# aghasemzadeh/OpenMPL

Hardware: AMD Instinct MI355X
Metric: poses/sec (V=4, J=17, batch=1024 per GPU) fp32 (higher is better)
Workload: dtype f32; 1 GPU; Human3.6M config: V=4 J=17 batch=1024 fp32, CHOSEN flag set, depth 12, DIM 32, heads 8; global_batch=1024, parallelism=single GPU

## Files before the change

### openmpl_amd/csrc/spt.hip

```cpp
#include <stdlib.h>

#include "common.hpp"

namespace mpl {

constexpr int SJ = 17;
constexpr int SD = 32;
constexpr int SH = 8;
constexpr int SEQ = 16;
constexpr int ROWS = SEQ * SJ;
constexpr int MT = ROWS / 16;
constexpr int XS = 36;
constexpr int QS = 100;
constexpr int NTHR = 512;
constexpr int NWAVE = NTHR / 64;
constexpr int SPT_LDS_BYTES = (ROWS * XS + ROWS * QS) * 4;

struct SptParams {
    const float* poses[MPL_MAX_VIEWS];
    const float* rays[MPL_MAX_VIEWS];
    const float* centers[MPL_MAX_VIEWS];
    const mpl_spt_set* sets;
    const float *snorm_w, *snorm_b;
    const float *pos3d_embed, *pos3d_view, *pos3d_lin_w, *pos3d_lin_b;
    const float *ray_w, *ray_b, *cfpt_w, *cfpt_b;
    float* xs;
    int B, V, in_ch, n_apps;
    unsigned flags;
    int c3;
    int spw;
    int abl;
    unsigned* err_host;
    unsigned char sched[MPL_MAX_APPS];
};

typedef const __attribute__((address_space(1))) float* gfp;
__device__ __forceinline__ gfp G(const float* p) { return (gfp)p; }
__device__ __forceinline__ float4 ld4(gfp p) {
    typedef float v4 __attribute__((ext_vector_type(4)));
    const v4 t = *reinterpret_cast<const __attribute__((address_space(1))) v4*>(p);
    return make_float4(t.x, t.y, t.z, t.w);
}

__device__ __forceinline__ void ln_frags(const float* X, int m, int li, int kq, const float4& g0, const float4& g1,
                                         const float4& b0, const float4& b1, float4& a0, float4& a1) {
    const float* xr = X + (m * 16 + li) * XS + 4 * kq;
    float4 x0 = ld4(xr), x1 = ld4(xr + 16);
    float s = ((x0.x + x0.y) + (x0.z + x0.w)) + ((x1.x + x1.y) + (x1.z + x1.w));
    s = xor16_add(s);
    s = xor32_add(s);
    const float mean = s * (1.0f / 32.0f);
    x0.x -= mean; x0.y -= mean; x0.z -= mean; x0.w -= mean;
    x1.x -= mean; x1.y -= mean; x1.z -= mean; x1.w -= mean;
    float ss = ((x0.x * x0.x + x0.y * x0.y) + (x0.z * x0.z + x0.w * x0.w)) +
               ((x1.x * x1.x + x1.y * x1.y) + (x1.z * x1.z + x1.w * x1.w));
    ss = xor16_add(ss);
    ss = xor32_add(ss);
    const float rstd = 1.0f / sqrtf(ss * (1.0f / 32.0f) + 1e-6f);
    a0.x = x0.x * rstd * g0.x + b0.x; a0.y = x0.y * rstd * g0.y + b0.y;
    a0.z = x0.z * rstd * g0.z + b0.z; a0.w = x0.w * rstd * g0.w + b0.w;
    a1.x = x1.x * rstd * g1.x + b1.x; a1.y = x1.y * rstd * g1.y + b1.y;
    a1.z = x1.z * rstd * g1.z + b1.z; a1.w = x1.w * rstd * g1.w + b1.w;
}

struct BlockFrags {
    float4 wq[6][2]; float bq[6];
    float4 wp[2][2]; float bp[2];
    float4 w1[4][2]; float b1[4];
    float4 w2[2][4]; float b2[2];
    float4 g1a, g1b, e1a, e1b;
    float4 g2a, g2b, e2a, e2b;
};

__device__ __forceinline__ void load_qkv_frags(const mpl_block_weights& bw, BlockFrags& F, int li, int kq) {
    F.g1a = ld4(G(bw.ln1_w) + 4 * kq); F.g1b = ld4(G(bw.ln1_w) + 16 + 4 * kq);
    F.e1a = ld4(G(bw.ln1_b) + 4 * kq); F.e1b = ld4(G(bw.ln1_b) + 16 + 4 * kq);
#pragma unroll
    for (int n = 0; n < 6; ++n) {
        const gfp wr = G(bw.qkv_w) + (n * 16 + li) * SD + 4 * kq;
        F.wq[n][0] = ld4(wr);
        F.wq[n][1] = ld4(wr + 16);
        F.bq[n] = G(bw.qkv_b)[n * 16 + li];
    }
}

__device__ __forceinline__ void load_proj_frags(const mpl_block_weights& bw, BlockFrags& F, int li, int kq) {
#pragma unroll
    for (int n = 0; n < 2; ++n) {
        const gfp wr = G(bw.proj_w) + (n * 16 + li) * SD + 4 * kq;
        F.wp[n][0] = ld4(wr);
        F.wp[n][1] = ld4(wr + 16);
        F.bp[n] = G(bw.proj_b)[n * 16 + li];
    }
}

__device__ __forceinline__ void load_fc1_frags(const mpl_block_weights& bw, BlockFrags& F, int li, int kq) {
    F.g2a = ld4(G(bw.ln2_w) + 4 * kq); F.g2b = ld4(G(bw.ln2_w) + 16 + 4 * kq);
    F.e2a = ld4(G(bw.ln2_b) + 4 * kq); F.e2b = ld4(G(bw.ln2_b) + 16 + 4 * kq);
#pragma unroll
    for (int n = 0; n < 4; ++n) {
        const gfp wr = G(bw.fc1_w) + (n * 16 + li) * SD + 4 * kq;
        F.w1[n][0] = ld4(wr);
        F.w1[n][1] = ld4(wr + 16);
        F.b1[n] = G(bw.fc1_b)[n * 16 + li];
    }
}

__device__ __forceinline__ void load_fc2_frags(const mpl_block_weights& bw, BlockFrags& F, int li, int kq) {
#pragma unroll
    for (int n = 0; n < 2; ++n) {
        const gfp wr = G(bw.fc2_w) + (n * 16 + li) * (2 * SD) + 4 * kq;
#pragma unroll
        for (int q = 0; q < 4; ++q) F.w2[n][q] = ld4(wr + 16 * q);
        F.b2[n] = G(bw.fc2_b)[n * 16 + li];
    }
}

constexpr int SPT_WB_VEC = 8192;
constexpr int SPT_WB_FLOATS = SPT_WB_VEC + 512;
constexpr int SPT_SMALL_ROWS = 144;
constexpr int SPT_SMALL_SPW = 8;
constexpr int SPT_SMALL_LDS_BYTES = (SPT_SMALL_ROWS * (XS + QS) + 2 * SPT_WB_FLOATS) * 4;
__device__ __forceinline__ const float* spt_uniform(const float* q) {
    const unsigned long long v = (unsigned long long)(uintptr_t)q;
    const unsigned lo = __builtin_amdgcn_readfirstlane((unsigned)v), hi = __builtin_amdgcn_readfirstlane((unsigned)(v >> 32));
    return reinterpret_cast<const float*>((uintptr_t)(((unsigned long long)hi << 32) | lo));
}
__device__ __forceinline__ void stage_block(const mpl_block_weights& bwv, float* wb, int wave, int lane, int w0, int nw) {
    if (wave < w0 || wave >= w0 + nw) return;
    const int li = lane & 15, kq = lane >> 4;
    struct { const float *qkv_w, *proj_w, *fc1_w, *fc2_w, *qkv_b, *proj_b, *fc1_b, *fc2_b, *ln1_w, *ln1_b, *ln2_w, *ln2_b; } bw;
    bw.qkv_w = spt_uniform(bwv.qkv_w); bw.proj_w = spt_uniform(bwv.proj_w); bw.fc1_w = spt_uniform(bwv.fc1_w); bw.fc2_w = spt_uniform(bwv.fc2_w);
    bw.qkv_b = spt_uniform(bwv.qkv_b); bw.proj_b = spt_uniform(bwv.proj_b); bw.fc1_b = spt_uniform(bwv.fc1_b); bw.fc2_b = spt_uniform(bwv.fc2_b);
    bw.ln1_w = spt_uniform(bwv.ln1_w); bw.ln1_b = spt_uniform(bwv.ln1_b); bw.ln2_w = spt_uniform(bwv.ln2_w); bw.ln2_b = spt_uniform(bwv.ln2_b);
    const unsigned lds0 = __builtin_amdgcn_readfirstlane((unsigned)(uintptr_t)(__attribute__((address_space(3))) float*)wb);
    for (int pc = wave - w0; pc < 34; pc += nw) {
        const float* src;
        bool on = true;
        if (pc < 12) src = bw.qkv_w + ((pc >> 1) * 16 + li) * SD + 16 * (pc & 1) + 4 * kq;
        else if (pc < 16) src = bw.proj_w + (((pc - 12) >> 1) * 16 + li) * SD + 16 * (pc & 1) + 4 * kq;
        else if (pc < 24) src = bw.fc1_w + (((pc - 16) >> 1) * 16 + li) * SD + 16 * (pc & 1) + 4 * kq;
        else if (pc < 32) src = bw.fc2_w + (((pc - 24) >> 2) * 16 + li) * (2 * SD) + 16 * (pc & 3) + 4 * kq;
        else if (pc == 32)
            src = lane < 24 ? bw.qkv_b + 4 * lane
                : lane < 32 ? bw.proj_b + 4 * (lane - 24)
                : lane < 48 ? bw.fc1_b + 4 * (lane - 32)
                : lane < 56 ? bw.fc2_b + 4 * (lane - 48) : bw.ln1_w + 4 * (lane - 56);
        else {
            src = lane < 8 ? bw.ln1_b + 4 * lane : lane < 16 ? bw.ln2_w + 4 * (lane - 8) : bw.ln2_b + 4 * (lane - 16);
            on = lane < 24;
        }
        if (on) dma16(src, lds0 + (unsigned)(pc * 1024));
    }
// ... 269 lines not shown
#pragma unroll
            for (int j = 0; j < SJ; ++j) {
                const float4 v = ld4(kb + j * QS + SD);
                const float pj = sc[j] * inv;
                o.x = fmaf(pj, v.x, o.x);
                o.y = fmaf(pj, v.y, o.y);
                o.z = fmaf(pj, v.z, o.z);
                o.w = fmaf(pj, v.w, o.w);
            }
            st4(Q + r * QS + 4 * h, o);
        }
        __syncthreads();
        stamp(1);

        if (!STAGED) {
#pragma unroll
            for (int n = 0; n < 2; ++n) { touch(F.wp[n][0]); touch(F.wp[n][1]); touch(F.bp[n]); }
            load_fc1_frags(bw, F, li, kq);
        }
        if (STAGED) {
            const int lo = (mt * 2 * wave) / NWAVE, hi = (mt * 2 * (wave + 1)) / NWAVE;
            for (int u = lo; u < hi && !(p.abl & 4); ++u) {
                const int m = u >> 1, n = u & 1;
                const float4 w0 = wb4(wb, 12 + 2 * n, lane), w1 = wb4(wb, 12 + 2 * n + 1, lane);
                const float bp = wb[SPT_WB_VEC + 96 + n * 16 + li];
                const float* ar = Q + (m * 16 + li) * QS + 4 * kq;
                const float4 a0 = ld4(ar), a1 = ld4(ar + 16);
                const f32x4 c = tile_k32(a0, a1, w0, w1);
                float* xd = X + (m * 16 + 4 * kq) * XS + n * 16 + li;
#pragma unroll
                for (int r = 0; r < 4; ++r) xd[r * XS] += c[r] + bp;
            }
        } else {
            const int lo = (mt * 2 * wave) / NWAVE, hi = (mt * 2 * (wave + 1)) / NWAVE;
            for (int m = lo >> 1; m <= ((hi - 1) >> 1) && !(p.abl & 4); ++m) {
                const float* ar = Q + (m * 16 + li) * QS + 4 * kq;
                const float4 a0 = ld4(ar), a1 = ld4(ar + 16);
#pragma unroll
                for (int n = 0; n < 2; ++n) {
                    const int u = 2 * m + n;
                    if (u < lo || u >= hi) continue;
                    const f32x4 c = tile_k32(a0, a1, F.wp[n][0], F.wp[n][1]);
                    float* xd = X + (m * 16 + 4 * kq) * XS + n * 16 + li;
#pragma unroll
                    for (int r = 0; r < 4; ++r) xd[r * XS] += c[r] + F.bp[n];
                }
            }
        }
        __syncthreads();
        stamp(2);

        if (!STAGED) {
#pragma unroll
            for (int n = 0; n < 4; ++n) { touch(F.w1[n][0]); touch(F.w1[n][1]); touch(F.b1[n]); }
            touch(F.g2a); touch(F.g2b); touch(F.e2a); touch(F.e2b);
            load_fc2_frags(bw, F, li, kq);
        }
        if (STAGED) {
            const int lo = (mt * 4 * wave) / NWAVE, hi = (mt * 4 * (wave + 1)) / NWAVE;
            const float4 g0 = wbv4(wb, 288, kq), g1 = wbv4(wb, 304, kq), e0 = wbv4(wb, 320, kq), e1 = wbv4(wb, 336, kq);
            float4 a0, a1;
            int m_have = -1;
            for (int u = lo; u < hi && !(p.abl & 4); ++u) {
                const int m = u >> 2, n = u & 3;
                const float4 w0 = wb4(wb, 16 + 2 * n, lane), w1 = wb4(wb, 16 + 2 * n + 1, lane);
                const float b1 = wb[SPT_WB_VEC + 128 + n * 16 + li];
                if (m != m_have) { ln_frags(X, m, li, kq, g0, g1, e0, e1, a0, a1); m_have = m; }
                const f32x4 c = tile_k32(a0, a1, w0, w1);
                float* qd = Q + (m * 16 + 4 * kq) * QS + n * 16 + li;
#pragma unroll
                for (int r = 0; r < 4; ++r) qd[r * QS] = (p.abl & 2) ? (c[r] + b1) : gelu_erf(c[r] + b1);
            }
        } else {
            const int lo = (mt * 4 * wave) / NWAVE, hi = (mt * 4 * (wave + 1)) / NWAVE;
            for (int m = lo >> 2; m <= ((hi - 1) >> 2) && !(p.abl & 4); ++m) {
                float4 a0, a1;
                ln_frags(X, m, li, kq, F.g2a, F.g2b, F.e2a, F.e2b, a0, a1);
#pragma unroll
                for (int n = 0; n < 4; ++n) {
                    const int u = 4 * m + n;
                    if (u < lo || u >= hi) continue;
                    const f32x4 c = tile_k32(a0, a1, F.w1[n][0], F.w1[n][1]);
                    float* qd = Q + (m * 16 + 4 * kq) * QS + n * 16 + li;
#pragma unroll
                    for (int r = 0; r < 4; ++r)
                        qd[r * QS] = (p.abl & 2) ? (c[r] + F.b1[n]) : gelu_erf(c[r] + F.b1[n]);
                }
            }
        }
        __syncthreads();
        stamp(3);

        if (!STAGED) {
#pragma unroll
            for (int n = 0; n < 2; ++n) {
#pragma unroll
                for (int q = 0; q < 4; ++q) touch(F.w2[n][q]);
                touch(F.b2[n]);
            }
            if (more) load_qkv_frags(bw_next, F, li, kq);
        }
        if (STAGED) {
            const int lo = (mt * 2 * wave) / NWAVE, hi = (mt * 2 * (wave + 1)) / NWAVE;
            for (int u = lo; u < hi && !(p.abl & 4); ++u) {
                const int m = u >> 1, n = u & 1;
                const float4 w0 = wb4(wb, 24 + 4 * n, lane), w1 = wb4(wb, 24 + 4 * n + 1, lane), w2 = wb4(wb, 24 + 4 * n + 2, lane),
                             w3 = wb4(wb, 24 + 4 * n + 3, lane);
                const float b2 = wb[SPT_WB_VEC + 192 + n * 16 + li];
                const float* ar = Q + (m * 16 + li) * QS + 4 * kq;
                const float4 a0 = ld4(ar), a1 = ld4(ar + 16), a2 = ld4(ar + 32), a3 = ld4(ar + 48);
                const f32x4 c = tile_k32(a0, a1, w0, w1) + tile_k32(a2, a3, w2, w3);
                float* xd = X + (m * 16 + 4 * kq) * XS + n * 16 + li;
#pragma unroll
                for (int r = 0; r < 4; ++r) xd[r * XS] += c[r] + b2;
            }
        } else {
            const int lo = (mt * 2 * wave) / NWAVE, hi = (mt * 2 * (wave + 1)) / NWAVE;
            for (int m = lo >> 1; m <= ((hi - 1) >> 1) && !(p.abl & 4); ++m) {
                const float* ar = Q + (m * 16 + li) * QS + 4 * kq;
                const float4 a0 = ld4(ar), a1 = ld4(ar + 16), a2 = ld4(ar + 32), a3 = ld4(ar + 48);
#pragma unroll
                for (int n = 0; n < 2; ++n) {
                    const int u = 2 * m + n;
                    if (u < lo || u >= hi) continue;
                    const f32x4 c = tile_k32(a0, a1, F.w2[n][0], F.w2[n][1]) + tile_k32(a2, a3, F.w2[n][2], F.w2[n][3]);
                    float* xd = X + (m * 16 + 4 * kq) * XS + n * 16 + li;
#pragma unroll
                    for (int r = 0; r < 4; ++r) xd[r * XS] += c[r] + F.b2[n];
                }
            }
        }
        if (STAGED) asm volatile("s_waitcnt vmcnt(0)" ::: "memory");
        __syncthreads();
        stamp(4);
        bw = bw_next;
        if (STAGED && app + 2 < p.n_apps) bw_next = bw_after;
    }

    if ((p.abl & 16) && lane == 0 && blockIdx.x < 32) {
        float* o = p.xs + (size_t)(blockIdx.x * NWAVE + wave) * 8;
        for (int k = 0; k < 6; ++k) o[k] = (float)ph[k];
        return;
    }
    if (p.abl & 16) return;
    spt_epilogue<false>(p, X, tid, view, b0, pose, ray, cen, nl, rows_live);
}

constexpr int ATS = 36;
constexpr int HS = 68;
constexpr int KV_F = SJ * SH * SEQ * 4;
constexpr int SPT3_RING_BYTES = (ROWS * XS + 2 * KV_F + ROWS * ATS) * 4;
constexpr int SPT3_LDS_BYTES = 160 * 1024;
constexpr int SPT3_HID_OFF = 3072;
constexpr int SPT3_Q_OFF = 20480;
constexpr int SPT3_NPAR = 456;
static_assert(SPT3_HID_OFF + ROWS * HS <= 2 * KV_F + ROWS * ATS, "HID does not fit its alias");
static_assert((SPT3_HID_OFF + ROWS * HS - 2 * KV_F) * 4 <= SPT3_Q_OFF, "HID reaches into the staged qkv weights");
static_assert(SPT3_Q_OFF + 12 * 1024 <= ROWS * ATS * 4, "staged qkv weights do not fit behind HID in ATT");
static_assert(SPT3_RING_BYTES + 8 * 1024 + 2 * SPT3_NPAR * 4 <= SPT3_LDS_BYTES, "spare LDS too small");
constexpr int SPT_PACK_QKV = 0, SPT_PACK_PROJ = 12 * 1024, SPT_PACK_FC1 = 16 * 1024, SPT_PACK_FC2 = 24 * 1024;
constexpr int SPT_PACK_VEC = 32 * 1024;
constexpr int SPT_PACK_BYTES = 48 * 1024;
constexpr int SPT_C_QKV = 0, SPT_C_PROJ = 96, SPT_C_FC1 = 128, SPT_C_FC2 = 192, SPT_NCOL = 224;
constexpr float SPT_SA = 1024.0f;
constexpr float SPT_QS = 0.5f * 1.4426950408889634f;

typedef _Float16 sf16x8 __attribute__((ext_vector_type(8)));
typedef float f32x2 __attribute__((ext_vector_type(2)));

__device__ __forceinline__ void spt_split2(const float (&x)[8], sf16x8& hi, sf16x8& lo) { ::mpl::split2_f16(x, hi, lo); }
__device__ inline float spt_window_scale(float v) {
    if (!(v > 0.f) || !(v < 3.0e38f)) return 1.0f;
    int e;
    (void)frexpf(32768.0f / v, &e);
    e = e - 1 < -100 ? -100 : (e - 1 > 100 ? 100 : e - 1);
    return ldexpf(1.0f, e);
}

__global__ __launch_bounds__(256) void spt_pack_kernel(const float* __restrict__ qkv_w, const float* __restrict__ qkv_b,
                                                        const float* __restrict__ ln1_w, const float* __restrict__ ln1_b,
                                                        const float* __restrict__ proj_w, const float* __restrict__ proj_b,
                                                        const float* __restrict__ fc1_w, const float* __restrict__ fc1_b,
                                                        const float* __restrict__ ln2_w, const float* __restrict__ ln2_b,
                                                        const float* __restrict__ fc2_w, const float* __restrict__ fc2_b,
                                                        char* __restrict__ dst, int fold_q) {
    __shared__ float Wf[8192];
    __shared__ float cn[SPT_NCOL], sw[SPT_NCOL], bnd[SPT_NCOL], scal[2];
    const int tid = threadIdx.x;
    for (int i = tid; i < 8192; i += 256) {
        float w;
        if (i < 3072) w = qkv_w[i] * ln1_w[i & 31];
        else if (i < 4096) w = proj_w[i - 3072];
        else if (i < 6144) w = fc1_w[i - 4096] * ln2_w[i & 31];
        else w = fc2_w[i - 6144];
        Wf[i] = w;
    }
    __syncthreads();
    if (tid < SPT_NCOL) {
        const int n = tid;
        const float *wr, *raw, *beta = nullptr;
        int K = 32;
        float bias;
        if (n < 96) { wr = Wf + n * 32; raw = qkv_w + n * 32; beta = ln1_b; bias = qkv_b[n]; }
        else if (n < 128) { wr = Wf + 3072 + (n - 96) * 32; raw = proj_w + (n - 96) * 32; bias = proj_b[n - 96]; }
        else if (n < 192) { wr = Wf + 4096 + (n - 128) * 32; raw = fc1_w + (n - 128) * 32; beta = ln2_b; bias = fc1_b[n - 128]; }
        else { wr = Wf + 6144 + (n - 192) * 64; raw = fc2_w + (n - 192) * 64; bias = fc2_b[n - 192]; K = 64; }
        float amax = 0.f;
        double ss = 0.0, c = (double)bias;
        for (int k = 0; k < K; ++k) {
            amax = fmaxf(amax, fabsf(wr[k]));
            ss += (double)wr[k] * (double)wr[k];
            if (beta) c += (double)raw[k] * (double)beta[k];
        }
        float s = 1.0f;
        if (amax > 0.f && amax < 3.0e38f) {
            int e;
            (void)frexpf(amax, &e);
            e = 14 - e;
            e = e < -100 ? -100 : (e > 100 ? 100 : e);
            s = ldexpf(1.0f, e);
        }
        cn[n] = (float)c;
        sw[n] = s;
        bnd[n] = beta ? (float)(sqrt(32.0) * sqrt(ss)) + fabsf((float)c) : 0.f;
    }
    __syncthreads();
    if (tid == 0) {
        float batt = 0.f, bhid = 0.f;
        for (int n = 64; n < 96; ++n) batt = fmaxf(batt, bnd[n]);
        for (int n = SPT_C_FC1; n < SPT_C_FC2; ++n) bhid = fmaxf(bhid, bnd[n]);
        scal[0] = spt_window_scale(batt);
        scal[1] = spt_window_scale(bhid);
    }
    __syncthreads();
    float* vec = reinterpret_cast<float*>(dst + SPT_PACK_VEC);
    if (tid < SPT_NCOL) {
        const int n = tid;
        float c = cn[n], sc;
        if (n < 96) sc = 1.0f / (SPT_SA * sw[n]);
        else if (n < 128) sc = 1.0f / (scal[0] * sw[n]);
        else if (n < 192) sc = 1.0f / (SPT_SA * sw[n]);
        else sc = 1.0f / (scal[1] * sw[n]);
        if (n < 32 && fold_q) { c *= SPT_QS; sc *= SPT_QS; }
        vec[n] = c;
        vec[SPT_NCOL + n] = sc;
    }
    if (tid < 8) vec[2 * SPT_NCOL + tid] = tid == 0 ? scal[0] : (tid == 1 ? 0.5f * scal[1] : 0.f);
    sf16x8* frag = reinterpret_cast<sf16x8*>(dst);
    for (int idx = tid; idx < 16 * 64; idx += 256) {
        const int lane = idx & 63, u = idx >> 6, li = lane & 15, kq = lane >> 4;
        const float* src;
        int n;
        if (u < 6) { n = 16 * u + li; src = Wf + n * 32 + 8 * kq; }
        else if (u < 8) { n = 16 * (u - 6) + li; src = Wf + 3072 + n * 32 + 8 * kq; n += SPT_C_PROJ; }
        else if (u < 12) { n = 16 * (u - 8) + li; src = Wf + 4096 + n * 32 + 8 * kq; n += SPT_C_FC1; }
        else { n = 16 * ((u - 12) >> 1) + li; src = Wf + 6144 + n * 64 + 32 * ((u - 12) & 1) + 8 * kq; n += SPT_C_FC2; }
        float x[8];
#pragma unroll
        for (int j = 0; j < 8; ++j) x[j] = src[j] * sw[n];
        sf16x8 hi, lo;
        spt_split2(x, hi, lo);
        frag[(size_t)(u * 2) * 64 + lane] = hi;
        frag[(size_t)(u * 2 + 1) * 64 + lane] = lo;
    }
}

int launch_spt_pack(const mpl_block_weights* bw_host, unsigned short* dst, int fold_q, hipStream_t s) {
    const mpl_block_weights* b = bw_host;
    if (!b || !dst || !b->qkv_w || !b->proj_w || !b->fc1_w || !b->fc2_w || !b->qkv_b || !b->proj_b || !b->fc1_b || !b->fc2_b ||
        !b->ln1_w || !b->ln1_b || !b->ln2_w || !b->ln2_b)
        return MPL_E_INVALID;
    ProfScope prof(MPL_K_PACK, s);
    hipLaunchKernelGGL(spt_pack_kernel, dim3(1), dim3(256), 0, s, b->qkv_w, b->qkv_b, b->ln1_w, b->ln1_b, b->proj_w, b->proj_b, b->fc1_w,
                       b->fc1_b, b->ln2_w, b->ln2_b, b->fc2_w, b->fc2_b, reinterpret_cast<char*>(dst), fold_q);
    return hip_check_launch();
}

size_t spt_pack_bytes() { return SPT_PACK_BYTES; }

__device__ __forceinline__ f32x4 mfma3(const sf16x8 (&w)[2], const sf16x8& ah, const sf16x8& al, f32x4 c) {
    c = __builtin_amdgcn_mfma_f32_16x16x32_f16(w[0], al, c, 0, 0, 0);
    c = __builtin_amdgcn_mfma_f32_16x16x32_f16(w[1], ah, c, 0, 0, 0);
    c = __builtin_amdgcn_mfma_f32_16x16x32_f16(w[0], ah, c, 0, 0, 0);
    return c;
}

template <int SS>
__global__ __launch_bounds__(NTHR, 1) void spt3_kernel(const SptParams p) {
    constexpr int RLIVE = SJ * SS;
    constexpr int MTS = (RLIVE + 15) / 16;
    constexpr int NT = (MTS + 3) / 4;
    extern __shared__ __attribute__((aligned(16))) float smem[];
    float* X = smem;
    float* Kb = smem + ROWS * XS;
    float* Vb = Kb + KV_F;
    float* ATT = Vb + KV_F;
    float* HID = Kb + SPT3_HID_OFF;
    char* S_W = reinterpret_cast<char*>(ATT + ROWS * ATS);
    float* S_PAR = reinterpret_cast<float*>(S_W + 8 * 1024);
    char* R_F1 = reinterpret_cast<char*>(Kb);
    char* R_Q = reinterpret_cast<char*>(ATT) + SPT3_Q_OFF;

    const int tid = threadIdx.x, lane = tid & 63;
    const int wave = __builtin_amdgcn_readfirstlane(tid >> 6);
    const int li = lane & 15, kq = lane >> 4;
    auto phase_sync = [&]() {
        asm volatile("s_waitcnt vmcnt(0)" ::: "memory");
        __syncthreads();
    };
    const int hg = wave & 1, part = wave >> 1;
    const int view = blockIdx.x % p.V;
    const int b0 = (blockIdx.x / p.V) * SS;
    const int sl = li % SS;
    const mpl_spt_set set = p.sets[(p.flags & MPL_F_MULTI_SPT) ? view : 0];
    const float* pose = p.poses[view];
    const float* ray = p.rays[view];
    const float* cen = p.centers[view];

    auto stage_w = [&](char* dst, const unsigned short* pack, int byte_off, int n_pieces) {
        const unsigned l0 = (unsigned)(uintptr_t)(__attribute__((address_space(3))) char*)dst;
        for (int i = wave; i < n_pieces; i += NWAVE)
            ::mpl::dma16(reinterpret_cast<const float*>(reinterpret_cast<const char*>(pack) + byte_off + i * 1024) + lane * 4,
                         l0 + (unsigned)(i * 1024));
    };
    auto load_par = [&](const mpl_block_weights& b) -> float4 {
        if (tid >= SPT3_NPAR / 4) return float4{0.f, 0.f, 0.f, 0.f};
        return ld4(G(reinterpret_cast<const float*>(reinterpret_cast<const char*>(b.qkv_w3) + SPT_PACK_VEC)) + 4 * tid);
    };
    auto store_par = [&](int app_of, const float4& v) {
        if (tid < SPT3_NPAR / 4) st4(S_PAR + (app_of & 1) * SPT3_NPAR + 4 * tid, v);
    };
    mpl_block_weights bw;
    if (p.n_apps > 0) {
        bw = set.blocks[p.sched[0] & 0x7f];
        stage_w(R_Q, bw.qkv_w3, SPT_PACK_QKV, 12);
    }
    const float4 par0 = p.n_apps > 0 ? load_par(bw) : float4{0.f, 0.f, 0.f, 0.f};
    spt_embed<true, SS>(p, set, X, tid, b0, pose, ray, cen, SS, MTS * 16);
    store_par(0, par0);
    phase_sync();

    auto load_w = [&](const char* region, int unit, sf16x8 (&w)[2]) {
        const sf16x8* g = reinterpret_cast<const sf16x8*>(region) + (size_t)unit * 2 * 64 + lane;
        w[0] = g[0];
        w[1] = g[64];
    };
    auto ln_frag = [&](int m, sf16x8& ah, sf16x8& al) {
        const float* xr = X + (m * 16 + li) * XS + 8 * kq;
        float4 x0 = ::mpl::ld4(xr), x1 = ::mpl::ld4(xr + 4);
        float sm = ((x0.x + x0.y) + (x0.z + x0.w)) + ((x1.x + x1.y) + (x1.z + x1.w));
        sm = ::mpl::xor32_add(::mpl::xor16_add(sm));
        const float mean = sm * (1.0f / 32.0f);
        x0.x -= mean; x0.y -= mean; x0.z -= mean; x0.w -= mean;
        x1.x -= mean; x1.y -= mean; x1.z -= mean; x1.w -= mean;
        float ss = ((x0.x * x0.x + x0.y * x0.y) + (x0.z * x0.z + x0.w * x0.w)) +
                   ((x1.x * x1.x + x1.y * x1.y) + (x1.z * x1.z + x1.w * x1.w));
        ss = ::mpl::xor32_add(::mpl::xor16_add(ss));
        const float rs = __builtin_amdgcn_rsqf(ss * (1.0f / 32.0f) + 1e-6f) * SPT_SA;
        const float y[8] = {x0.x * rs, x0.y * rs, x0.z * rs, x0.w * rs, x1.x * rs, x1.y * rs, x1.z * rs, x1.w * rs};
        spt_split2(y, ah, al);
    };
    auto raw_frag = [&](const float* rowp, sf16x8& ah, sf16x8& al) {
        const float4 x0 = ::mpl::ld4(rowp), x1 = ::mpl::ld4(rowp + 4);
        const float y[8] = {x0.x, x0.y, x0.z, x0.w, x1.x, x1.y, x1.z, x1.w};
        spt_split2(y, ah, al);
    };

    for (int app = 0; app < p.n_apps; ++app) {
        const bool weighted = (p.sched[app] & 0x80) != 0;
        bw = set.blocks[p.sched[app] & 0x7f];
        const unsigned short* pack = bw.qkv_w3;
        const float* par = S_PAR + (app & 1) * SPT3_NPAR;
        stage_w(S_W, pack, SPT_PACK_PROJ, 4);
        {
            sf16x8 wq[3][2];
            float4 bq[3], sq[3];
#pragma unroll
            for (int c = 0; c < 3; ++c) {
                load_w(R_Q, 2 * c + hg, wq[c]);
                bq[c] = ::mpl::ld4(par + SPT_C_QKV + 32 * c + 16 * hg + 4 * kq);
                sq[c] = ::mpl::ld4(par + SPT_NCOL + SPT_C_QKV + 32 * c + 16 * hg + 4 * kq);
            }
            float4 q[NT];
#pragma unroll
            for (int t = 0; t < NT; ++t) {
                q[t] = float4{0.f, 0.f, 0.f, 0.f};
                if (part + 4 * t < MTS && !(p.abl & 8)) {
                    const int m = part + 4 * t;
                    const int j = (16 * m + li) / SS;
                    const bool live = 16 * m + li < RLIVE;
                    sf16x8 ah, al;
                    ln_frag(m, ah, al);
                    const f32x4 z = {0.f, 0.f, 0.f, 0.f};
                    const f32x4 cq = mfma3(wq[0], ah, al, z), ck = mfma3(wq[1], ah, al, z), cv = mfma3(wq[2], ah, al, z);
                    q[t] = float4{fmaf(cq[0], sq[0].x, bq[0].x), fmaf(cq[1], sq[0].y, bq[0].y), fmaf(cq[2], sq[0].z, bq[0].z),
                                  fmaf(cq[3], sq[0].w, bq[0].w)};
                    const int h = 4 * hg + kq;
                    const float kx = fmaf(ck[0], sq[1].x, bq[1].x), ky = fmaf(ck[1], sq[1].y, bq[1].y);
                    const float kz = fmaf(ck[2], sq[1].z, bq[1].z), kw = fmaf(ck[3], sq[1].w, bq[1].w);
                    if (live && j < SJ - 1) {
                        float* kp = Kb + ((((j >> 1) * 2) * SH + h) * SS + sl) * 4 + (j & 1);
                        kp[0] = kx;
                        kp[2] = ky;
                        kp[SH * SS * 4] = kz;
                        kp[SH * SS * 4 + 2] = kw;
                    } else if (live) {
                        st4(Kb + (SJ - 1) * SH * SS * 4 + (h * SS + sl) * 4, float4{kx, ky, kz, kw});
                    }
                    if (live)
                        st4(Vb + ((j * SH + h) * SS + sl) * 4, float4{fmaf(cv[0], sq[2].x, bq[2].x), fmaf(cv[1], sq[2].y, bq[2].y),
                                                                       fmaf(cv[2], sq[2].z, bq[2].z), fmaf(cv[3], sq[2].w, bq[2].w)});
                }
            }
            phase_sync();
            if (!(p.abl & 1)) {
                const int h = 4 * hg + kq;
                float sc[NT][SJ];
#pragma unroll
                for (int jp = 0; jp < SJ / 2; ++jp) {
                    const float4 k01 = ::mpl::ld4(Kb + (((jp * 2) * SH + h) * SS + sl) * 4);
                    const float4 k23 = ::mpl::ld4(Kb + (((jp * 2 + 1) * SH + h) * SS + sl) * 4);
                    const f32x2 kx = {k01.x, k01.y}, ky = {k01.z, k01.w}, kz = {k23.x, k23.y}, kw = {k23.z, k23.w};
#pragma unroll
                    for (int t = 0; t < NT; ++t) {
                        const f32x2 qx = {q[t].x, q[t].x}, qy = {q[t].y, q[t].y}, qz = {q[t].z, q[t].z}, qw = {q[t].w, q[t].w};
                        f32x2 s2 = qx * kx;
                        s2 = __builtin_elementwise_fma(qy, ky, s2);
                        s2 = __builtin_elementwise_fma(qz, kz, s2);
                        s2 = __builtin_elementwise_fma(qw, kw, s2);
                        sc[t][2 * jp] = s2[0];
                        sc[t][2 * jp + 1] = s2[1];
                    }
                }
                {
                    const float4 k = ::mpl::ld4(Kb + (SJ - 1) * SH * SS * 4 + (h * SS + sl) * 4);
#pragma unroll
                    for (int t = 0; t < NT; ++t)
                        sc[t][SJ - 1] = fmaf(q[t].w, k.w, fmaf(q[t].z, k.z, fmaf(q[t].y, k.y, q[t].x * k.x)));
                }
                const float s_att = par[2 * SPT_NCOL];
                float inv[NT];
#pragma unroll
                for (int t = 0; t < NT; ++t) {
                    float mx = sc[t][0];
#pragma unroll
                    for (int j = 1; j < SJ; ++j) mx = fmaxf(mx, sc[t][j]);
                    float l = 0.f;
#pragma unroll
                    for (int j = 0; j < SJ; ++j) {
                        sc[t][j] = __builtin_amdgcn_exp2f(sc[t][j] - mx);
                        l += sc[t][j];
                    }
                    inv[t] = __builtin_amdgcn_rcpf(l) * s_att;
                    if (weighted) {
                        const int b = b0 + sl, r = 16 * (part + 4 * t) + li;
                        inv[t] *= (b < p.B && r < RLIVE) ? pose[((size_t)b * SJ + r / SS) * 3 + 2] : 0.f;
                    }
                }
                float4 o[NT];
#pragma unroll
                for (int t = 0; t < NT; ++t) o[t] = float4{0.f, 0.f, 0.f, 0.f};
#pragma unroll
                for (int j = 0; j < SJ; ++j) {
                    const float4 v = ::mpl::ld4(Vb + ((j * SH + h) * SS + sl) * 4);
#pragma unroll
                    for (int t = 0; t < NT; ++t) {
                        const float pj = sc[t][j];
                        o[t].x = fmaf(pj, v.x, o[t].x);
                        o[t].y = fmaf(pj, v.y, o[t].y);
                        o[t].z = fmaf(pj, v.z, o[t].z);
                        o[t].w = fmaf(pj, v.w, o[t].w);
                    }
                }
#pragma unroll
                for (int t = 0; t < NT; ++t) {
                    o[t] = float4{o[t].x * inv[t], o[t].y * inv[t], o[t].z * inv[t], o[t].w * inv[t]};
                    if (weighted) {
                        const float big = fmaxf(fmaxf(fabsf(o[t].x), fabsf(o[t].y)), fmaxf(fabsf(o[t].z), fabsf(o[t].w)));
                        if (!(big <= 65000.f)) {
                            const float qn = __builtin_nanf("");
                            o[t] = float4{qn, qn, qn, qn};
                            if (p.err_host) __hip_atomic_fetch_or(p.err_host, 2u, __ATOMIC_RELAXED, __HIP_MEMORY_SCOPE_SYSTEM);
                        }
                    }
                }
#pragma unroll
                for (int t = 0; t < NT; ++t)
                    if (part + 4 * t < MTS) st4(ATT + ((part + 4 * t) * 16 + li) * ATS + 4 * h, o[t]);
            }
        }
        phase_sync();
        {
            stage_w(R_F1, pack, SPT_PACK_FC1, 8);
            sf16x8 wp[2][2];
            float4 bp[2], sp[2];
#pragma unroll
            for (int n = 0; n < 2; ++n) {
                load_w(S_W, n, wp[n]);
                bp[n] = ::mpl::ld4(par + SPT_C_PROJ + 16 * n + 4 * kq);
                sp[n] = ::mpl::ld4(par + SPT_NCOL + SPT_C_PROJ + 16 * n + 4 * kq);
            }
            const int lo = (MTS * 2 * wave) / NWAVE, hi = (MTS * 2 * (wave + 1)) / NWAVE;
            for (int m = lo >> 1; m <= ((hi - 1) >> 1) && !(p.abl & 32); ++m) {
                sf16x8 ah, al;
                raw_frag(ATT + (m * 16 + li) * ATS + 8 * kq, ah, al);
#pragma unroll
                for (int n = 0; n < 2; ++n) {
                    const int u = 2 * m + n;
                    if (u < lo || u >= hi) continue;
                    const f32x4 c = mfma3(wp[n], ah, al, f32x4{0.f, 0.f, 0.f, 0.f});
                    float* xd = X + (m * 16 + li) * XS + 16 * n + 4 * kq;
                    const float4 x = ::mpl::ld4(xd);
                    st4(xd, float4{x.x + fmaf(c[0], sp[n].x, bp[n].x), x.y + fmaf(c[1], sp[n].y, bp[n].y),
                                   x.z + fmaf(c[2], sp[n].z, bp[n].z), x.w + fmaf(c[3], sp[n].w, bp[n].w)});
                }
            }
        }
        phase_sync();
        {
            stage_w(S_W, pack, SPT_PACK_FC2, 8);
            sf16x8 w1[4][2];
            float4 b1[4], s1[4];
#pragma unroll
            for (int n = 0; n < 4; ++n) {
                load_w(R_F1, n, w1[n]);
                b1[n] = ::mpl::ld4(par + SPT_C_FC1 + 16 * n + 4 * kq);
                s1[n] = ::mpl::ld4(par + SPT_NCOL + SPT_C_FC1 + 16 * n + 4 * kq);
            }
            const float hs = par[2 * SPT_NCOL + 1];
            const int lo = (MTS * 4 * wave) / NWAVE, hi = (MTS * 4 * (wave + 1)) / NWAVE;
            for (int m = lo >> 2; m <= ((hi - 1) >> 2) && !(p.abl & 64); ++m) {
                sf16x8 ah, al;
                ln_frag(m, ah, al);
#pragma unroll
                for (int n = 0; n < 4; ++n) {
                    const int u = 4 * m + n;
                    if (u < lo || u >= hi) continue;
                    const f32x4 c = mfma3(w1[n], ah, al, f32x4{0.f, 0.f, 0.f, 0.f});
                    st4(HID + (m * 16 + li) * HS + 16 * n + 4 * kq,
                        float4{gelu_as_scaled(fmaf(c[0], s1[n].x, b1[n].x), hs), gelu_as_scaled(fmaf(c[1], s1[n].y, b1[n].y), hs),
                               gelu_as_scaled(fmaf(c[2], s1[n].z, b1[n].z), hs), gelu_as_scaled(fmaf(c[3], s1[n].w, b1[n].w), hs)});
                }
            }
        }
        phase_sync();
        {
            float4 parn = float4{0.f, 0.f, 0.f, 0.f};
            if (app + 1 < p.n_apps) {
                const mpl_block_weights bn = set.blocks[p.sched[app + 1] & 0x7f];
                stage_w(R_Q, bn.qkv_w3, SPT_PACK_QKV, 12);
                parn = load_par(bn);
            }
            sf16x8 w2[2][2][2];
            float4 b2[2], s2[2];
#pragma unroll
            for (int n = 0; n < 2; ++n) {
                load_w(S_W, 2 * n, w2[n][0]);
                load_w(S_W, 2 * n + 1, w2[n][1]);
                b2[n] = ::mpl::ld4(par + SPT_C_FC2 + 16 * n + 4 * kq);
                s2[n] = ::mpl::ld4(par + SPT_NCOL + SPT_C_FC2 + 16 * n + 4 * kq);
            }
            const int lo = (MTS * 2 * wave) / NWAVE, hi = (MTS * 2 * (wave + 1)) / NWAVE;
            for (int m = lo >> 1; m <= ((hi - 1) >> 1) && !(p.abl & 128); ++m) {
                sf16x8 ah0, al0, ah1, al1;
                raw_frag(HID + (m * 16 + li) * HS + 8 * kq, ah0, al0);
                raw_frag(HID + (m * 16 + li) * HS + 32 + 8 * kq, ah1, al1);
#pragma unroll
                for (int n = 0; n < 2; ++n) {
                    const int u = 2 * m + n;
                    if (u < lo || u >= hi) continue;
                    f32x4 c = mfma3(w2[n][0], ah0, al0, f32x4{0.f, 0.f, 0.f, 0.f});
                    c = mfma3(w2[n][1], ah1, al1, c);
                    float* xd = X + (m * 16 + li) * XS + 16 * n + 4 * kq;
                    const float4 x = ::mpl::ld4(xd);
                    st4(xd, float4{x.x + fmaf(c[0], s2[n].x, b2[n].x), x.y + fmaf(c[1], s2[n].y, b2[n].y),
                                   x.z + fmaf(c[2], s2[n].z, b2[n].z), x.w + fmaf(c[3], s2[n].w, b2[n].w)});
                }
            }
            if (app + 1 < p.n_apps) store_par(app + 1, parn);
        }
        phase_sync();
    }
    spt_epilogue<true, SS>(p, X, tid, view, b0, pose, ray, cen, SS, MTS * 16);
}

__device__ __forceinline__ void d32_ln_split(const float4& a0, const float4& a1, sf16x8& ah, sf16x8& al) {
    float4 x0 = a0, x1 = a1;
    float sm = ((x0.x + x0.y) + (x0.z + x0.w)) + ((x1.x + x1.y) + (x1.z + x1.w));
    sm = xor32_add(xor16_add(sm));
    const float mean = sm * (1.0f / 32.0f);
    x0.x -= mean; x0.y -= mean; x0.z -= mean; x0.w -= mean;
    x1.x -= mean; x1.y -= mean; x1.z -= mean; x1.w -= mean;
    float ss = ((x0.x * x0.x + x0.y * x0.y) + (x0.z * x0.z + x0.w * x0.w)) + ((x1.x * x1.x + x1.y * x1.y) + (x1.z * x1.z + x1.w * x1.w));
    ss = xor32_add(xor16_add(ss));
    const float rs = __builtin_amdgcn_rsqf(ss * (1.0f / 32.0f) + 1e-6f) * SPT_SA;
    const float y[8] = {x0.x * rs, x0.y * rs, x0.z * rs, x0.w * rs, x1.x * rs, x1.y * rs, x1.z * rs, x1.w * rs};
    spt_split2(y, ah, al);
}
__device__ __forceinline__ void d32_load_w(const char* pack, int unit, int lane, sf16x8 (&w)[2]) {
    const sf16x8* g = reinterpret_cast<const sf16x8*>(pack) + (size_t)unit * 2 * 64 + lane;
    w[0] = g[0];
    w[1] = g[64];
}

__global__ __launch_bounds__(512) void d32_qkv_kernel(const float* __restrict__ x, int M, const char* __restrict__ pack,
                                                       float* __restrict__ qkv) {
    const int lane = threadIdx.x & 63, li = lane & 15, kq = lane >> 4;
    const int gw = blockIdx.x * 8 + (threadIdx.x >> 6), nw = gridDim.x * 8;
    const float* vec = reinterpret_cast<const float*>(pack + SPT_PACK_VEC);
    sf16x8 wq[6][2];
    float4 cq[6], sq[6];
#pragma unroll
    for (int n = 0; n < 6; ++n) {
        d32_load_w(pack, n, lane, wq[n]);
        cq[n] = ld4(vec + SPT_C_QKV + 16 * n + 4 * kq);
        sq[n] = ld4(vec + SPT_NCOL + SPT_C_QKV + 16 * n + 4 * kq);
    }
    const int n_tiles = (M + 15) / 16;
    auto rows_of = [&](int tile, float4& a0, float4& a1) {
        const int r = tile * 16 + li;
        const float* xr = x + (size_t)(r < M ? r : M - 1) * SD + 8 * kq;
        a0 = ld4(xr);
        a1 = ld4(xr + 4);
    };
    float4 n0 = {0.f, 0.f, 0.f, 0.f}, n1 = n0;
    if (gw < n_tiles) rows_of(gw, n0, n1);
    for (int tile = gw; tile < n_tiles; tile += nw) {
        const int row = tile * 16 + li;
        const bool ok = row < M;
        const float4 c0 = n0, c1 = n1;
        if (tile + nw < n_tiles) rows_of(tile + nw, n0, n1);
        sf16x8 ah, al;
        d32_ln_split(c0, c1, ah, al);
        float* o = qkv + (size_t)row * (3 * SD) + 4 * kq;
#pragma unroll
        for (int n = 0; n < 6; ++n) {
            const f32x4 c = mfma3(wq[n], ah, al, f32x4{0.f, 0.f, 0.f, 0.f});
            if (ok) st4(o + 16 * n, float4{fmaf(c[0], sq[n].x, cq[n].x), fmaf(c[1], sq[n].y, cq[n].y), fmaf(c[2], sq[n].z, cq[n].z),
                                           fmaf(c[3], sq[n].w, cq[n].w)});
        }
    }
// ... 193 lines not shown
```

Measured before the change: 878,200 poses/s.

## Precompute LayerNorm fragments once into LDS and split attention by live tiles

Each wave now computes its share of LayerNorm fp16 hi/lo fragments once and stores them in the ATT region of LDS. The QKV staged weights move to the start of the K buffer to make room. Previously the fragments were recomputed redundantly by the head-group/part waves, and the QKV loop now reads them after an extra barrier. Attention is split into compile-time chunks of at most three tiles and dispatched by the number of live tiles per wave. This avoids computing dead tiles and lowers register pressure from the score arrays. The cost is an extra __syncthreads and changed LDS aliasing, which risks overlapping buffers.

```diff
diff --git a/openmpl_amd/csrc/spt.hip b/openmpl_amd/csrc/spt.hip
--- a/openmpl_amd/csrc/spt.hip
+++ b/openmpl_amd/csrc/spt.hip
@@ -1,4 +1,6 @@
 #include <stdlib.h>
+
+#include <type_traits>
 
 #include "common.hpp"
 
@@ -574,11 +576,10 @@
 constexpr int SPT3_RING_BYTES = (ROWS * XS + 2 * KV_F + ROWS * ATS) * 4;
 constexpr int SPT3_LDS_BYTES = 160 * 1024;
 constexpr int SPT3_HID_OFF = 3072;
-constexpr int SPT3_Q_OFF = 20480;
 constexpr int SPT3_NPAR = 456;
 static_assert(SPT3_HID_OFF + ROWS * HS <= 2 * KV_F + ROWS * ATS, "HID does not fit its alias");
-static_assert((SPT3_HID_OFF + ROWS * HS - 2 * KV_F) * 4 <= SPT3_Q_OFF, "HID reaches into the staged qkv weights");
-static_assert(SPT3_Q_OFF + 12 * 1024 <= ROWS * ATS * 4, "staged qkv weights do not fit behind HID in ATT");
+static_assert(12 * 1024 <= SPT3_HID_OFF * 4, "staged qkv weights reach into HID");
+static_assert(MT * 2048 <= ROWS * ATS * 4, "LayerNorm fragments do not fit in ATT");
 static_assert(SPT3_RING_BYTES + 8 * 1024 + 2 * SPT3_NPAR * 4 <= SPT3_LDS_BYTES, "spare LDS too small");
 constexpr int SPT_PACK_QKV = 0, SPT_PACK_PROJ = 12 * 1024, SPT_PACK_FC1 = 16 * 1024, SPT_PACK_FC2 = 24 * 1024;
 constexpr int SPT_PACK_VEC = 32 * 1024;
@@ -721,7 +722,8 @@
     char* S_W = reinterpret_cast<char*>(ATT + ROWS * ATS);
     float* S_PAR = reinterpret_cast<float*>(S_W + 8 * 1024);
     char* R_F1 = reinterpret_cast<char*>(Kb);
-    char* R_Q = reinterpret_cast<char*>(ATT) + SPT3_Q_OFF;
+    char* R_Q = reinterpret_cast<char*>(Kb);
+    sf16x8* FR = reinterpret_cast<sf16x8*>(ATT);
 
     const int tid = threadIdx.x, lane = tid & 63;
     const int wave = __builtin_amdgcn_readfirstlane(tid >> 6);
@@ -803,6 +805,19 @@
                 bq[c] = ::mpl::ld4(par + SPT_C_QKV + 32 * c + 16 * hg + 4 * kq);
                 sq[c] = ::mpl::ld4(par + SPT_NCOL + SPT_C_QKV + 32 * c + 16 * hg + 4 * kq);
             }
+            if (!(p.abl & 8)) {
+#pragma unroll
+                for (int i = 0; i < 3; ++i) {
+                    const int m = i < 2 ? wave + NWAVE * i : 2 * NWAVE + (NWAVE - 1 - wave);
+                    if (m < MTS) {
+                        sf16x8 ah, al;
+                        ln_frag(m, ah, al);
+                        FR[(2 * m) * 64 + lane] = ah;
+                        FR[(2 * m + 1) * 64 + lane] = al;
+                    }
+                }
+            }
+            __syncthreads();
             float4 q[NT];
 #pragma unroll
             for (int t = 0; t < NT; ++t) {
@@ -811,8 +826,7 @@
                     const int m = part + 4 * t;
                     const int j = (16 * m + li) / SS;
                     const bool live = 16 * m + li < RLIVE;
-                    sf16x8 ah, al;
-                    ln_frag(m, ah, al);
+                    const sf16x8 ah = FR[(2 * m) * 64 + lane], al = FR[(2 * m + 1) * 64 + lane];
                     const f32x4 z = {0.f, 0.f, 0.f, 0.f};
                     const f32x4 cq = mfma3(wq[0], ah, al, z), ck = mfma3(wq[1], ah, al, z), cv = mfma3(wq[2], ah, al, z);
                     q[t] = float4{fmaf(cq[0], sq[0].x, bq[0].x), fmaf(cq[1], sq[0].y, bq[0].y), fmaf(cq[2], sq[0].z, bq[0].z),
@@ -837,78 +851,92 @@
             phase_sync();
             if (!(p.abl & 1)) {
                 const int h = 4 * hg + kq;
-                float sc[NT][SJ];
-#pragma unroll
-                for (int jp = 0; jp < SJ / 2; ++jp) {
-                    const float4 k01 = ::mpl::ld4(Kb + (((jp * 2) * SH + h) * SS + sl) * 4);
-                    const float4 k23 = ::mpl::ld4(Kb + (((jp * 2 + 1) * SH + h) * SS + sl) * 4);
-                    const f32x2 kx = {k01.x, k01.y}, ky = {k01.z, k01.w}, kz = {k23.x, k23.y}, kw = {k23.z, k23.w};
-#pragma unroll
-                    for (int t = 0; t < NT; ++t) {
-                        const f32x2 qx = {q[t].x, q[t].x}, qy = {q[t].y, q[t].y}, qz = {q[t].z, q[t].z}, qw = {q[t].w, q[t].w};
-                        f32x2 s2 = qx * kx;
-                        s2 = __builtin_elementwise_fma(qy, ky, s2);
-                        s2 = __builtin_elementwise_fma(qz, kz, s2);
-                        s2 = __builtin_elementwise_fma(qw, kw, s2);
-                        sc[t][2 * jp] = s2[0];
-                        sc[t][2 * jp + 1] = s2[1];
-                    }
-                }
-                {
-                    const float4 k = ::mpl::ld4(Kb + (SJ - 1) * SH * SS * 4 + (h * SS + sl) * 4);
-#pragma unroll
-                    for (int t = 0; t < NT; ++t)
-                        sc[t][SJ - 1] = fmaf(q[t].w, k.w, fmaf(q[t].z, k.z, fmaf(q[t].y, k.y, q[t].x * k.x)));
-                }
                 const float s_att = par[2 * SPT_NCOL];
-                float inv[NT];
-#pragma unroll
-                for (int t = 0; t < NT; ++t) {
-                    float mx = sc[t][0];
-#pragma unroll
-                    for (int j = 1; j < SJ; ++j) mx = fmaxf(mx, sc[t][j]);
-                    float l = 0.f;
-#pragma unroll
-                    for (int j = 0; j < SJ; ++j) {
-                        sc[t][j] = __builtin_amdgcn_exp2f(sc[t][j] - mx);
-                        l += sc[t][j];
-                    }
-                    inv[t] = __builtin_amdgcn_rcpf(l) * s_att;
-                    if (weighted) {
-                        const int b = b0 + sl, r = 16 * (part + 4 * t) + li;
-                        inv[t] *= (b < p.B && r < RLIVE) ? pose[((size_t)b * SJ + r / SS) * 3 + 2] : 0.f;
-                    }
-                }
-                float4 o[NT];
-#pragma unroll
-                for (int t = 0; t < NT; ++t) o[t] = float4{0.f, 0.f, 0.f, 0.f};
-#pragma unroll
-                for (int j = 0; j < SJ; ++j) {
-                    const float4 v = ::mpl::ld4(Vb + ((j * SH + h) * SS + sl) * 4);
-#pragma unroll
-                    for (int t = 0; t < NT; ++t) {
-                        const float pj = sc[t][j];
-                        o[t].x = fmaf(pj, v.x, o[t].x);
-                        o[t].y = fmaf(pj, v.y, o[t].y);
-                        o[t].z = fmaf(pj, v.z, o[t].z);
-                        o[t].w = fmaf(pj, v.w, o[t].w);
-                    }
-                }
-#pragma unroll
-                for (int t = 0; t < NT; ++t) {
-                    o[t] = float4{o[t].x * inv[t], o[t].y * inv[t], o[t].z * inv[t], o[t].w * inv[t]};
-                    if (weighted) {
-                        const float big = fmaxf(fmaxf(fabsf(o[t].x), fabsf(o[t].y)), fmaxf(fabsf(o[t].z), fabsf(o[t].w)));
-                        if (!(big <= 65000.f)) {
-                            const float qn = __builtin_nanf("");
-                            o[t] = float4{qn, qn, qn, qn};
-                            if (p.err_host) __hip_atomic_fetch_or(p.err_host, 2u, __ATOMIC_RELAXED, __HIP_MEMORY_SCOPE_SYSTEM);
+                auto attend = [&](auto t0c, auto t1c) {
+                    constexpr int T0 = decltype(t0c)::value, T1 = decltype(t1c)::value;
+                    if constexpr (T1 > T0) {
+                        constexpr int TN = T1 - T0;
+                        float sc[TN][SJ];
+#pragma unroll
+                        for (int jp = 0; jp < SJ / 2; ++jp) {
+                            const float4 k01 = ::mpl::ld4(Kb + (((jp * 2) * SH + h) * SS + sl) * 4);
+                            const float4 k23 = ::mpl::ld4(Kb + (((jp * 2 + 1) * SH + h) * SS + sl) * 4);
+                            const f32x2 kx = {k01.x, k01.y}, ky = {k01.z, k01.w}, kz = {k23.x, k23.y}, kw = {k23.z, k23.w};
+#pragma unroll
+                            for (int u = 0; u < TN; ++u) {
+                                const float4& qt = q[T0 + u];
+                                const f32x2 qx = {qt.x, qt.x}, qy = {qt.y, qt.y}, qz = {qt.z, qt.z}, qw = {qt.w, qt.w};
+                                f32x2 s2 = qx * kx;
+                                s2 = __builtin_elementwise_fma(qy, ky, s2);
+                                s2 = __builtin_elementwise_fma(qz, kz, s2);
+                                s2 = __builtin_elementwise_fma(qw, kw, s2);
+                                sc[u][2 * jp] = s2[0];
+                                sc[u][2 * jp + 1] = s2[1];
+                            }
+                        }
+                        {
+                            const float4 k = ::mpl::ld4(Kb + (SJ - 1) * SH * SS * 4 + (h * SS + sl) * 4);
+#pragma unroll
+                            for (int u = 0; u < TN; ++u) {
+                                const float4& qt = q[T0 + u];
+                                sc[u][SJ - 1] = fmaf(qt.w, k.w, fmaf(qt.z, k.z, fmaf(qt.y, k.y, qt.x * k.x)));
+                            }
+                        }
+                        float inv[TN];
+#pragma unroll
+                        for (int u = 0; u < TN; ++u) {
+                            float mx = sc[u][0];
+#pragma unroll
+                            for (int j = 1; j < SJ; ++j) mx = fmaxf(mx, sc[u][j]);
+                            float l = 0.f;
+#pragma unroll
+                            for (int j = 0; j < SJ; ++j) {
+                                sc[u][j] = __builtin_amdgcn_exp2f(sc[u][j] - mx);
+                                l += sc[u][j];
+                            }
+                            inv[u] = __builtin_amdgcn_rcpf(l) * s_att;
+                            if (weighted) {
+                                const int b = b0 + sl, r = 16 * (part + 4 * (T0 + u)) + li;
+                                inv[u] *= (b < p.B && r < RLIVE) ? pose[((size_t)b * SJ + r / SS) * 3 + 2] : 0.f;
+                            }
+                        }
+                        float4 o[TN];
+#pragma unroll
+                        for (int u = 0; u < TN; ++u) o[u] = float4{0.f, 0.f, 0.f, 0.f};
+#pragma unroll
+                        for (int j = 0; j < SJ; ++j) {
+                            const float4 v = ::mpl::ld4(Vb + ((j * SH + h) * SS + sl) * 4);
+#pragma unroll
+                            for (int u = 0; u < TN; ++u) {
+                                const float pj = sc[u][j];
+                                o[u].x = fmaf(pj, v.x, o[u].x);
+                                o[u].y = fmaf(pj, v.y, o[u].y);
+                                o[u].z = fmaf(pj, v.z, o[u].z);
+                                o[u].w = fmaf(pj, v.w, o[u].w);
+                            }
+                        }
+#pragma unroll
+                        for (int u = 0; u < TN; ++u) {
+                            o[u] = float4{o[u].x * inv[u], o[u].y * inv[u], o[u].z * inv[u], o[u].w * inv[u]};
+                            if (weighted) {
+                                const float big = fmaxf(fmaxf(fabsf(o[u].x), fabsf(o[u].y)), fmaxf(fabsf(o[u].z), fabsf(o[u].w)));
+                                if (!(big <= 65000.f)) {
+                                    const float qn = __builtin_nanf("");
+                                    o[u] = float4{qn, qn, qn, qn};
+                                    if (p.err_host) __hip_atomic_fetch_or(p.err_host, 2u, __ATOMIC_RELAXED, __HIP_MEMORY_SCOPE_SYSTEM);
+                                }
+                            }
+                            st4(ATT + ((part + 4 * (T0 + u)) * 16 + li) * ATS + 4 * h, o[u]);
                         }
                     }
-                }
-#pragma unroll
-                for (int t = 0; t < NT; ++t)
-                    if (part + 4 * t < MTS) st4(ATT + ((part + 4 * t) * 16 + li) * ATS + 4 * h, o[t]);
+                };
+                using I0 = std::integral_constant<int, 0>;
+                constexpr int NA = NT < 3 ? NT : 3;
+                const int nv = part < MTS ? (MTS - part + 3) / 4 : 0;
+                if (nv >= NA) attend(I0{}, std::integral_constant<int, NA>{});
+                else if (nv == NA - 1) attend(I0{}, std::integral_constant<int, NA - 1>{});
+                if (nv >= NT) attend(std::integral_constant<int, NA>{}, std::integral_constant<int, NT>{});
+                else if (nv == NT - 1) attend(std::integral_constant<int, NA>{}, std::integral_constant<int, NT - 1>{});
             }
         }
         phase_sync();
```

New measurement: 885,700 poses/s, median of 6. No clear change (+0.8%).
